# balaji1312/cassnat_asr_public

Measured on AMD Instinct MI355X. Metric: utterances_per_sec, higher is better.
Workload: dtype bf16; 1 GPU; BASELINE configs[1]: CASS-NAT 12L-enc / 1+3+2 dec blocks, d_model 256, 4 heads, d_ff 2048, V 5000, greedy NAST; 32 utterances x 1000 frames x 80 fbank per GPU per step; batch_per_gpu=32, frames=1000, feat_dim=80, global_batch=32, parallelism=utterance-sharded x1, decode_pipelines_per_gpu=2, batches_per_engine_pass=10, utterances_per_engine_pass=320, row_predictions=208, row_predictions_missed=0

## Files before the change

cassnat_asr_public_amd/csrc/attention.hip:

```cpp
#include <cstdlib>

#include <cstdio>
#include <cstdlib>

#include "kernels.h"

struct AttnParams {
    const unsigned char* Q;
    const unsigned char* K;
    const unsigned char* V;
    void* O;
    long long ldq_b, ldk_b, ldv_b;
    int ldo;
    int H, Lq, Lk;
    const unsigned char* keymask;
    int kv_mod;
    int stamps;
    const int* kv_index;
    const int* klen;
    int o_blk;
    int q_blk, kv_blk;
    int q_col, k_col, v_col, q_n, kv_n;
    const int* kcap;
    int kcap_stride;
    const int* iv;
    int iv_stride;
    int causal;
    float scale;
    const float* rel_pos;
    const float* rel_u;
    const float* rel_v;
    int rel_R, ld_pos;
    const int* row_off;
    int kv_packed;
    const unsigned char* Y;
    const unsigned char* W;
    const float* bt;
};

template <typename T> struct AttnCfg;
template <> struct AttnCfg<bf16> {
    static constexpr int KROW = 128;
    static constexpr int VROW = 192;
    static constexpr int CPR = 8;
    __device__ static int swz(int row) { return (row >> 1) & 7; }
};
template <> struct AttnCfg<float> {
    static constexpr int KROW = 256;
    static constexpr int VROW = 256;
    static constexpr int CPR = 16;
    __device__ static int swz(int row) { return row & 15; }
};

template <> struct AttnCfg<split_t> {
    static constexpr int KROW = 256;
    static constexpr int VROW = 192;
    static constexpr int CPR = 16;
    __device__ static int swz(int row) { return row & 15; }
};

__device__ long long attn_stamps[8];
#define AT_STAMP(i) if (p.stamps && blockIdx.x == 0 && blockIdx.y == gridDim.y - 1 && blockIdx.z == gridDim.z - 1 && threadIdx.x == 0) attn_stamps[i] = (long long)__builtin_amdgcn_s_memtime();

template <typename T, int NW, bool RES, bool REL = false, bool PK = false, bool PROJ = false>
__global__ __launch_bounds__(64 * NW, (RES && NW == 8) ? 4 : ((__is_same(T, split_t) && NW == 4 && !REL) ? 2 : 1)) void attention_kernel(AttnParams p) {
    typedef AttnCfg<T> Cfg;
    typedef typename Frag<T>::type frag_t;
    constexpr bool SPLIT = __is_same(T, split_t);
    static_assert(!SPLIT || !RES, "split-bf16 attention: the staged forms only");
    static_assert(!PROJ || (RES && NW == 8 && !REL && !PK && sizeof(T) == 2), "the projecting form: resident, 8 waves, 16-bit operands");
    constexpr int KROW = Cfg::KROW, CPR = Cfg::CPR;
    constexpr int VROW = RES ? 128 : Cfg::VROW;
    constexpr int KT_BYTES = 64 * KROW, VT_BYTES = (SPLIT ? 2 : 1) * 64 * VROW, NRES = RES ? 4 : 1;
    constexpr int NF = SPLIT ? 4 : KROW / 32;
    constexpr int NT = 64 * NW;
    constexpr int ST_IT = 64 * CPR / NT;

    __shared__ __attribute__((aligned(16))) unsigned char Ks_all[NRES * KT_BYTES];
    __shared__ __attribute__((aligned(16))) unsigned char Vs_all[NRES * VT_BYTES];
    __shared__ __attribute__((aligned(16))) unsigned int Ms_all[NRES * 16];
    __shared__ unsigned int Mplain[NRES];

    const int tid = threadIdx.x, lane = tid & 63, wave = tid >> 6;
    const int half = lane >> 5, l31 = lane & 31;
    int b = blockIdx.z, h = blockIdx.y;
    if constexpr (PROJ) {
        const int id = blockIdx.y + 4 * blockIdx.z, grp = id >> 5, r = id & 31;
        if (grp < ((int)gridDim.z >> 3)) {
            b = grp * 8 + (r & 7);
            h = r >> 3;
        }
    }
    AT_STAMP(0)
    const long long q0 = PK ? (long long)p.row_off[b] : (long long)b * p.Lq;
    const int Lq = PK ? p.row_off[b + 1] - p.row_off[b] : p.Lq;
    if constexpr (PK) {
        if ((int)blockIdx.x * (32 * NW) >= Lq) return;
    }
    const int q_row = blockIdx.x * (32 * NW) + wave * 32 + l31;
    const bool wave_active = (blockIdx.x * (32 * NW) + wave * 32) < Lq;
    const int qc = q_row < Lq ? q_row : Lq - 1;

    frag_t qf[NF];
    {
        const unsigned char* qp = p.Q + (q0 + qc) * p.ldq_b + (long long)h * KROW;
        if constexpr (PROJ) {
            (void)qp;
        } else if constexpr (SPLIT) {
#pragma unroll
            for (int s = 0; s < NF; ++s) {
                const unsigned char* c = qp + (s >> 1) * 128 + (2 * (s & 1) + half) * 16;
                qf[s].hi = as_frag<bf16>(ld16(c));
                qf[s].lo = as_frag<bf16>(ld16(c + 64));
            }
        } else if constexpr (PK) {
            const long long qm = q0 + qc;
#pragma unroll
            for (int s = 0; s < NF; ++s) {
                const unsigned char* src = qp + (2 * s + half) * 16;
                src = p.q_blk ? p.Q + cn_blk16_off(qm, p.q_col + h * 64 + (2 * s + half) * 8, p.q_n) : src;
                qf[s] = as_frag<T>(ld16(src));
            }
        } else if (p.q_blk) {
            const long long qm = q0 + qc;
#pragma unroll
            for (int s = 0; s < NF; ++s) qf[s] = as_frag<T>(ld16(p.Q + cn_blk16_off(qm, p.q_col + h * 64 + (2 * s + half) * 8, p.q_n)));
        } else {
#pragma unroll
            for (int s = 0; s < NF; ++s) qf[s] = as_frag<T>(ld16(qp + (2 * s + half) * 16));
        }
    }
    if constexpr (PROJ) {
        typedef unsigned u32x4 __attribute__((ext_vector_type(4)));
        const long long ym = q0 + qc;
        int y_half = half;
        asm volatile("" : "+v"(y_half));
        const int y_lane = ((y_half << 5) + (int)(ym & 31)) * 16;
        const unsigned char* yb = p.Y + (ym >> 5) * 16384 + y_lane;
        const int key = wave * 32 + l31;
        bf16x8 yf[16];
#pragma unroll
        for (int ks = 0; ks < 16; ++ks) yf[ks] = as_frag<bf16>(ld16(yb + ks * 1024));
        uint4 wr[4];
        auto fetch = [&](int tile) {
            const uint4* src = reinterpret_cast<const uint4*>(p.W) + (long long)tile * 1024 + tid;
#pragma unroll
            for (int i = 0; i < 4; ++i) wr[i] = src[NT * i];
        };
        auto put = [&]() {
#pragma unroll
            for (int i = 0; i < 4; ++i) st16(Ks_all + (tid + NT * i) * 16, wr[i]);
        };
        auto project = [&](int tile, int d, u32x4& o_0, u32x4& o_1) {
            f32x16 a;
#pragma unroll
            for (int g = 0; g < 4; ++g) {
                const f32x4 v = *reinterpret_cast<const f32x4*>(p.bt + 32 * tile + 8 * g + 4 * half);
#pragma unroll
                for (int e = 0; e < 4; ++e) a[4 * g + e] = v[e];
            }
#pragma unroll
            for (int ks = 0; ks < 16; ++ks)
                a = CN_MFMA16(as_frag<bf16>(ld16(Ks_all + d * 16384 + ks * 1024 + lane * 16)), yf[ks], a, 0, 0, 0);
#pragma unroll
            for (int gp = 0; gp < 2; ++gp) {
                bf16x4 o0, o1;
#pragma unroll
                for (int e = 0; e < 4; ++e) {
                    o0[e] = (bf16)a[8 * gp + e];
                    o1[e] = (bf16)a[8 * gp + 4 + e];
                }
                const uint2 lo_ = __builtin_bit_cast(uint2, o0), hi_ = __builtin_bit_cast(uint2, o1);
                const auto s0_ = __builtin_amdgcn_permlane32_swap(lo_.x, hi_.x, false, false);
                const auto s1_ = __builtin_amdgcn_permlane32_swap(lo_.y, hi_.y, false, false);
                (gp ? o_1 : o_0) = u32x4{s0_[0], s1_[0], s0_[1], s1_[1]};
            }
        };
        u32x4 pk[4];
        fetch(16 + 2 * h);
        put();
        __syncthreads();
#pragma unroll
        for (int d = 0; d < 2; ++d) {
            project(16 + 2 * h + d, d, pk[0], pk[1]);
#pragma unroll
            for (int c = 0; c < 2; ++c)
                *reinterpret_cast<u32x4*>(Vs_all + key * 128 + (((2 * (2 * d + c) + half) ^ (((key >> 1) & 1) << 2)) << 4)) = pk[c];
        }
        __syncthreads();
        fetch(2 * h);
        put();
        __syncthreads();
#pragma unroll
        for (int d = 0; d < 2; ++d) {
            project(2 * h + d, d, pk[0], pk[1]);
            qf[2 * d] = __builtin_bit_cast(bf16x8, pk[0]);
            qf[2 * d + 1] = __builtin_bit_cast(bf16x8, pk[1]);
        }
        __syncthreads();
        fetch(8 + 2 * h);
        put();
        __syncthreads();
        project(8 + 2 * h, 0, pk[0], pk[1]);
        project(8 + 2 * h + 1, 1, pk[2], pk[3]);
        __syncthreads();
#pragma unroll
        for (int c = 0; c < 4; ++c)
            *reinterpret_cast<u32x4*>(Ks_all + key * KROW + (((2 * c + half) ^ Cfg::swz(key)) << 4)) = pk[c];
        AT_STAMP(1)
    }
    constexpr int REL_N = REL ? 64 : 1;
    __shared__ float rel_tab[REL ? 64 * 64 : 1];
    __shared__ float rel_bias[REL ? NW : 1][32][REL_N];
    if constexpr (REL) {
        constexpr int E = SPLIT ? 8 : Frag<T>::ELEMS;
        const int nr = 2 * p.rel_R + 1;
        for (int i = tid; i < nr * 64; i += NT) rel_tab[i] = p.rel_pos[(long long)(i >> 6) * p.ld_pos + h * 64 + (i & 63)];
        __syncthreads();
        auto dim_of = [&](int s, int j) -> int {
            if constexpr (SPLIT) return 32 * (s >> 1) + 16 * (s & 1) + 8 * half + j;
            else return (2 * s + half) * E + j;
        };
        float qv[NF][E];
#pragma unroll
        for (int s = 0; s < NF; ++s)
#pragma unroll
            for (int j = 0; j < E; ++j) {
                const int dim = dim_of(s, j);
                if constexpr (SPLIT) {
                    const float q = (float)qf[s].hi[j] + (float)qf[s].lo[j];
                    qv[s][j] = q + p.rel_v[h * 64 + dim];
                    const float qu = q + p.rel_u[h * 64 + dim];
                    const bf16 hi = (bf16)qu;
                    qf[s].hi[j] = hi;
                    qf[s].lo[j] = (bf16)(qu - (float)hi);
                } else {
                    const float q = to_f32(qf[s][j]);
                    qv[s][j] = q + p.rel_v[h * 64 + dim];
                    qf[s][j] = from_f32<T>(q + p.rel_u[h * 64 + dim]);
                }
            }
        for (int r = 0; r < nr; ++r) {
            float acc = 0.f;
#pragma unroll
            for (int s = 0; s < NF; ++s)
#pragma unroll
                for (int j = 0; j < E; ++j) acc = fmaf(qv[s][j], rel_tab[r * 64 + dim_of(s, j)], acc);
            acc += __shfl_xor(acc, 32);
            if (half == 0) rel_bias[wave][l31][r] = acc;
        }
        __syncthreads();
    }
    int iv_s1 = 0, iv_e1 = 0, iv_s2 = 0, iv_e2 = 0;
    if (p.iv) {
        const int4 r = *reinterpret_cast<const int4*>(p.iv + ((long long)b * p.iv_stride + qc) * 4);
        iv_s1 = r.x;
        iv_e1 = r.y;
        iv_s2 = r.z;
        iv_e2 = r.w;
    }
    const int klen = p.klen ? p.klen[b] : p.Lk;
    unsigned char* Ks = Ks_all;
    unsigned char* Vs = Vs_all;
    unsigned int* Ms = Ms_all;

    uint4 k_reg[ST_IT], v_reg[ST_IT];
    const int bk = p.kv_index ? p.kv_index[b] : (p.kv_mod > 0 ? b % p.kv_mod : b);
    const bool kpk = PK && p.kv_packed;
    const long long k0 = kpk ? (long long)p.row_off[bk] : (long long)bk * p.Lk;
    const int krows = kpk ? p.row_off[bk + 1] - p.row_off[bk] : p.Lk;
    int kcap = p.kcap ? p.kcap[(long long)bk * p.kcap_stride] : p.Lk;
    if (krows < kcap) kcap = krows;
    const int kvalid = kcap < p.Lk ? kcap : p.Lk;
    const int nkt = kvalid > 0 ? (kvalid + 63) / 64 : 1;
    const unsigned char* kbase = p.K + k0 * p.ldk_b + (long long)h * KROW;
    const unsigned char* vbase = p.V + k0 * p.ldv_b + (long long)h * KROW;
    auto load_tile = [&](int kt) {
#pragma unroll
        for (int i = 0; i < ST_IT; ++i) {
            const int cidx = tid + NT * i;
            const int row = cidx / CPR, ch = cidx % CPR;
            const int key = kt * 64 + row;
            if (key < krows) {
                if (p.kv_blk) {
                    const long long km = k0 + key;
                    k_reg[i] = ld16(p.K + cn_blk16_off(km, p.k_col + h * 64 + ch * 8, p.kv_n));
                    v_reg[i] = ld16(p.V + cn_blk16_off(km, p.v_col + h * 64 + ch * 8, p.kv_n));
                } else {
                    k_reg[i] = ld16(kbase + (long long)key * p.ldk_b + ch * 16);
                    v_reg[i] = ld16(vbase + (long long)key * p.ldv_b + ch * 16);
                }
            } else {
                k_reg[i] = make_uint4(0, 0, 0, 0);
                v_reg[i] = make_uint4(0, 0, 0, 0);
            }
        }
    };
    auto store_tile = [&](int kt) {
#pragma unroll
        for (int i = 0; i < ST_IT; ++i) {
            const int cidx = tid + NT * i;
            const int row = cidx / CPR, ch = cidx % CPR;
            st16(Ks + row * KROW + ((ch ^ Cfg::swz(row)) << 4), k_reg[i]);
            if constexpr (SPLIT)
                st16(Vs + ((ch >> 2) & 1) * 64 * VROW + row * VROW + ((((ch >> 3) << 2) | (ch & 3)) << 4), v_reg[i]);
            else
                st16(Vs + row * VROW + (ch << 4), v_reg[i]);
        }
        if (tid < 64) {
            const int key = kt * 64 + tid;
            unsigned char code = 2;
            if (key < kcap) {
                bool ok = key < klen;
                if (p.keymask) ok = ok && p.keymask[(long long)bk * p.Lk + key] != 0;
                code = ok ? 1 : 0;
            }
            reinterpret_cast<unsigned char*>(Ms)[tid] = code;
            const unsigned long long bad0 = __ballot(code == 0), bad2 = __ballot(code == 2);
            if (tid == 0) Mplain[0] = 1u | (bad2 != 0ull ? 2u : 0u) | (bad0 != 0ull ? 4u : 0u);
        }
    };

    f32x16 o_acc[2];
#pragma unroll
    for (int d = 0; d < 2; ++d)
#pragma unroll
        for (int r = 0; r < 16; ++r) o_acc[d][r] = 0.f;
    float m_run = CN_NEG_FILL, l_run = 0.f;

    if constexpr (RES) {
        const int wave_u = __builtin_amdgcn_readfirstlane(wave);
        const int r8 = lane >> 3, cp = lane & 7;
        for (int piece = wave_u; !PROJ && piece < nkt * 16; piece += NW) {
            const int kt2 = piece >> 4, is_v = (piece >> 3) & 1, j = piece & 7;
            const int row = 8 * j + r8;
            int key = kt2 * 64 + row;
            if (key >= krows) key = krows - 1;
            const int chunk = is_v ? (cp ^ (((row >> 1) & 1) << 2)) : (cp ^ Cfg::swz(row));
            const unsigned char* src;
            if (p.kv_blk)
                src = (is_v ? p.V : p.K) + cn_blk16_off(k0 + key, (is_v ? p.v_col : p.k_col) + h * 64 + chunk * 8, p.kv_n);
            else
                src = is_v ? vbase + (long long)key * p.ldv_b + (chunk << 4) : kbase + (long long)key * p.ldk_b + (chunk << 4);
            unsigned char* dst = (is_v ? Vs_all + kt2 * VT_BYTES : Ks_all + kt2 * KT_BYTES) + j * 1024;
            __builtin_amdgcn_global_load_lds((const __attribute__((address_space(1))) void*)src,
                                             (__attribute__((address_space(3))) void*)dst, 16, 0, 0);
        }
        if constexpr (!PROJ) AT_STAMP(1)
        if (tid < NRES) Mplain[tid] = 1;
        __syncthreads();
        for (int i = tid; i < nkt * 64; i += NT) {
            unsigned char code = 2;
            if (i < kcap) {
                bool ok = i < klen;
                if (p.keymask) ok = ok && p.keymask[(long long)bk * p.Lk + i] != 0;
                code = ok ? 1 : 0;
            }
            reinterpret_cast<unsigned char*>(Ms_all)[i] = code;
            if (code != 1) atomicOr(&Mplain[i >> 6], code == 2 ? 2u : 4u);
        }
        asm volatile("s_waitcnt vmcnt(0)" ::: "memory");
        __syncthreads();
        AT_STAMP(2)
    } else {
        load_tile(0);
    }
    for (int kt = 0; kt < nkt; ++kt) {
        if constexpr (RES) {
            Ks = Ks_all + kt * KT_BYTES;
            Vs = Vs_all + kt * VT_BYTES;
            Ms = Ms_all + kt * 16;
        } else {
            __syncthreads();
            store_tile(kt);
            __syncthreads();
            if (kt + 1 < nkt) load_tile(kt + 1);
        }
        if (!wave_active) continue;

        const unsigned tile_class = Mplain[RES ? kt : 0];
        const bool simple = !REL && !p.iv && !p.causal && (tile_class & 4u) == 0;
#pragma unroll
        for (int sub = 0; sub < 2; ++sub) {
            if (simple && kt * 64 + sub * 32 >= kcap) continue;
            f32x16 sc;
#pragma unroll
            for (int r = 0; r < 16; ++r) sc[r] = 0.f;
            {
                const int row = sub * 32 + l31;
#pragma unroll
                for (int s = 0; s < NF; ++s) {
                    if constexpr (SPLIT) {
                        const int chunk = (s >> 1) * 8 + 2 * (s & 1) + half;
                        split_frag kf;
                        kf.hi = as_frag<bf16>(ld16(Ks + row * KROW + ((chunk ^ Cfg::swz(row)) << 4)));
                        kf.lo = as_frag<bf16>(ld16(Ks + row * KROW + (((chunk + 4) ^ Cfg::swz(row)) << 4)));
                        sc = mfma_frag(kf, qf[s], sc);
                    } else {
                        const int chunk = 2 * s + half;
                        const frag_t kf = as_frag<T>(ld16(Ks + row * KROW + ((chunk ^ Cfg::swz(row)) << 4)));
                        sc = mfma_frag(kf, qf[s], sc);
                    }
                }
            }
            float psum = 0.f, alpha;
            const bool plain = simple && kt * 64 + sub * 32 + 32 <= kcap;
            if (simple) {
                float tmax;
                if (plain) {
                    tmax = sc[0];
#pragma unroll
                    for (int r = 1; r < 16; ++r) tmax = fmaxf(tmax, sc[r]);
                } else {
                    const int k0 = kt * 64 + sub * 32 + 4 * half;
                    tmax = -INFINITY;
#pragma unroll
                    for (int r = 0; r < 16; ++r) {
                        sc[r] = k0 + 8 * (r >> 2) + (r & 3) < kcap ? sc[r] : -INFINITY;
                        tmax = fmaxf(tmax, sc[r]);
                    }
                }
                tmax = xhalf_max(tmax) * p.scale;
                const float m_new = fmaxf(m_run, tmax);
                alpha = __expf(m_run - m_new);
                m_run = m_new;
                const float c2 = p.scale * 1.44269504088896340736f, mb = m_new * 1.44269504088896340736f;
#pragma unroll
                for (int r = 0; r < 16; ++r) {
                    const float pv = __builtin_amdgcn_exp2f(fmaf(sc[r], c2, -mb));
                    sc[r] = pv;
                    psum += pv;
                }
            } else {
                float tmax = -INFINITY;
#pragma unroll
                for (int g = 0; g < 4; ++g) {
                    const unsigned int mw = Ms[sub * 8 + 2 * g + half];
#pragma unroll
                    for (int e = 0; e < 4; ++e) {
                        const int r = 4 * g + e;
                        const int key = kt * 64 + sub * 32 + 8 * g + 4 * half + e;
                        const unsigned int code = (mw >> (8 * e)) & 0xffu;
                        bool ok = code == 1u;
                        if (p.iv) ok = ok && ((key >= iv_s1 && key < iv_e1) || (key >= iv_s2 && key < iv_e2));
                        if (p.causal) ok = ok && key <= q_row;
                        float v = sc[r];
                        if constexpr (REL) {
                            int rd = key - q_row;
                            rd = rd < -p.rel_R ? -p.rel_R : (rd > p.rel_R ? p.rel_R : rd);
                            v += rel_bias[wave][l31][rd + p.rel_R];
                        }
                        v = ok ? v : CN_NEG_FILL;
                        v = code == 2u ? -INFINITY : v;
                        sc[r] = v;
                        tmax = fmaxf(tmax, ok ? v * p.scale : v);
                    }
                }
                tmax = xhalf_max(tmax);
                const float m_new = fmaxf(m_run, tmax);
                alpha = __expf(m_run - m_new);
                m_run = m_new;
                const float c2 = p.scale * 1.44269504088896340736f, mb = m_new * 1.44269504088896340736f;
                const float p_fill = __expf(CN_NEG_FILL - m_new);
#pragma unroll
                for (int r = 0; r < 16; ++r) {
                    const float v = sc[r];
                    float pv = __builtin_amdgcn_exp2f(fmaf(v, c2, -mb));
                    pv = v == CN_NEG_FILL ? p_fill : pv;
                    pv = v == -INFINITY ? 0.f : pv;
                    sc[r] = pv;
                    psum += pv;
                }
            }
            l_run = l_run * alpha + psum;
            if (!__all(alpha == 1.f)) {
#pragma unroll
                for (int d = 0; d < 2; ++d)
#pragma unroll
                    for (int r = 0; r < 16; ++r) o_acc[d][r] *= alpha;
            }

            if constexpr (SPLIT) {
                const int i16 = lane & 15, g1 = (lane >> 4) & 1;
                typedef short s16x8 __attribute__((ext_vector_type(8)));
#pragma unroll
                for (int s = 0; s < 2; ++s) {
                    bf16x8 ph, pl;
#pragma unroll
                    for (int j = 0; j < 8; ++j) {
                        ph[j] = (bf16)sc[8 * s + j];
                        pl[j] = (bf16)(sc[8 * s + j] - (float)ph[j]);
                    }
                    const int key0 = sub * 32 + 16 * s + 4 * half + (i16 >> 2);
#pragma unroll
                    for (int d = 0; d < 2; ++d) {
                        bf16x8 vf[2];
#pragma unroll
                        for (int pl_ = 0; pl_ < 2; ++pl_) {
                            const unsigned char* a1 = Vs + pl_ * 64 * VROW + key0 * VROW + (32 * d + 16 * g1 + 4 * (i16 & 3)) * 2;
                            const s16x4 r1 = __builtin_amdgcn_ds_read_tr16_b64_v4i16((s16x4 __attribute__((address_space(3)))*)(a1));
                            const s16x4 r2 = __builtin_amdgcn_ds_read_tr16_b64_v4i16((s16x4 __attribute__((address_space(3)))*)(a1 + 8 * VROW));
                            s16x8 cat;
                            cat[0] = r1[0]; cat[1] = r1[1]; cat[2] = r1[2]; cat[3] = r1[3];
                            cat[4] = r2[0]; cat[5] = r2[1]; cat[6] = r2[2]; cat[7] = r2[3];
                            vf[pl_] = __builtin_bit_cast(bf16x8, cat);
                        }
                        o_acc[d] = CN_MFMA16(vf[1], ph, o_acc[d], 0, 0, 0);
                        o_acc[d] = CN_MFMA16(vf[0], pl, o_acc[d], 0, 0, 0);
                        o_acc[d] = CN_MFMA16(vf[0], ph, o_acc[d], 0, 0, 0);
                    }
                }
            } else if constexpr (sizeof(T) == 2) {
                const int i16 = lane & 15, g1 = (lane >> 4) & 1;
#pragma unroll
                for (int s = 0; s < 2; ++s) {
                    bf16x8 pb;
#pragma unroll
                    for (int j = 0; j < 8; ++j) pb[j] = (bf16)sc[8 * s + j];
                    const int key0 = sub * 32 + 16 * s + 4 * half + (i16 >> 2);
#pragma unroll
                    for (int d = 0; d < 2; ++d) {
                        const int dd = RES ? (d ^ ((i16 >> 3) & 1)) : d;
                        const unsigned char* a1 = Vs + key0 * VROW + (32 * dd + 16 * g1 + 4 * (i16 & 3)) * 2;
                        const s16x4 r1 = __builtin_amdgcn_ds_read_tr16_b64_v4i16(
                            (s16x4 __attribute__((address_space(3)))*)(a1));
                        const s16x4 r2 = __builtin_amdgcn_ds_read_tr16_b64_v4i16(
                            (s16x4 __attribute__((address_space(3)))*)(a1 + 8 * VROW));
                        typedef short s16x8 __attribute__((ext_vector_type(8)));
                        s16x8 cat;
                        cat[0] = r1[0]; cat[1] = r1[1]; cat[2] = r1[2]; cat[3] = r1[3];
                        cat[4] = r2[0]; cat[5] = r2[1]; cat[6] = r2[2]; cat[7] = r2[3];
                        const bf16x8 vf = __builtin_bit_cast(bf16x8, cat);
                        o_acc[d] = CN_MFMA16(vf, pb, o_acc[d], 0, 0, 0);
                    }
                }
            } else {
#pragma unroll
                for (int r = 0; r < 16; ++r) {
                    const int key_local = sub * 32 + acc_row(r, lane);
                    const float* vrow = reinterpret_cast<const float*>(Vs + key_local * VROW);
#pragma unroll
                    for (int d = 0; d < 2; ++d)
                        o_acc[d] = __builtin_amdgcn_mfma_f32_32x32x2f32(vrow[32 * d + l31], sc[r], o_acc[d], 0, 0, 0);
                }
            }
        }
    }

    AT_STAMP(3)
    if (!wave_active) return;
    const float l_tot = xhalf_sum(l_run);
    const float inv = (REL && m_run == CN_NEG_FILL) ? 0.f : 1.f / l_tot;
    if constexpr (sizeof(T) == 2) {
        typedef unsigned u32x4 __attribute__((ext_vector_type(4)));
        T* orow = reinterpret_cast<T*>(p.O) + (q0 + qc) * p.ldo + h * 64 + 8 * half;
#pragma unroll
        for (int d = 0; d < 2; ++d) {
#pragma unroll
            for (int gp = 0; gp < 2; ++gp) {
                bf16x4 o0, o1;
#pragma unroll
                for (int e = 0; e < 4; ++e) {
                    o0[e] = (bf16)(o_acc[d][8 * gp + e] * inv);
                    o1[e] = (bf16)(o_acc[d][8 * gp + 4 + e] * inv);
                }
                const uint2 lo_ = __builtin_bit_cast(uint2, o0), hi_ = __builtin_bit_cast(uint2, o1);
                const auto s0_ = __builtin_amdgcn_permlane32_swap(lo_.x, hi_.x, false, false);
                const auto s1_ = __builtin_amdgcn_permlane32_swap(lo_.y, hi_.y, false, false);
                if (q_row < Lq) {
                    if (p.o_blk) {
                        const long long om = q0 + q_row;
                        unsigned char* ob = reinterpret_cast<unsigned char*>(p.O) +
                                            ((om >> 5) * (p.ldo >> 4) + (4 * h + 2 * d + gp)) * 1024 + ((half << 5) + (int)(om & 31)) * 16;
                        *reinterpret_cast<u32x4*>(ob) = u32x4{s0_[0], s1_[0], s0_[1], s1_[1]};
                    } else {
                        *reinterpret_cast<u32x4*>(orow + 32 * d + 16 * gp) = u32x4{s0_[0], s1_[0], s0_[1], s1_[1]};
                    }
                }
            }
        }
        return;
    }
    if (q_row < Lq) {
        T* orow = reinterpret_cast<T*>(p.O) + (q0 + q_row) * p.ldo + h * 64;
#pragma unroll
        for (int d = 0; d < 2; ++d) {
#pragma unroll
            for (int g = 0; g < 4; ++g) {
                const int dk0 = 32 * d + 8 * g + 4 * half;
                if constexpr (SPLIT) {
                    float o[4];
#pragma unroll
                    for (int e = 0; e < 4; ++e) o[e] = o_acc[d][4 * g + e] * inv;
                    bf16x4 hi, lo;
                    cn_split4(o, hi, lo);
                    unsigned char* ob = reinterpret_cast<unsigned char*>(orow) + cn_split_off((size_t)dk0);
                    *reinterpret_cast<bf16x4*>(ob) = hi;
                    *reinterpret_cast<bf16x4*>(ob + 64) = lo;
                } else if constexpr (sizeof(T) == 2) {
                    bf16x4 o;
#pragma unroll
                    for (int e = 0; e < 4; ++e) o[e] = (bf16)(o_acc[d][4 * g + e] * inv);
                    *reinterpret_cast<bf16x4*>(orow + dk0) = o;
                } else {
                    f32x4 o;
#pragma unroll
                    for (int e = 0; e < 4; ++e) o[e] = o_acc[d][4 * g + e] * inv;
                    *reinterpret_cast<f32x4*>(orow + dk0) = o;
                }
            }
        }
    }
    AT_STAMP(4)
}

int attention_print_stamps() {
    long long h[8];
    CN_HIP_CHECK(hipMemcpyFromSymbol(h, HIP_SYMBOL(attn_stamps), sizeof(h)));
    static const char* names[] = {"", "Q fragments + K/V requests", "K/V landed + mask codes", "key-tile loop", "normalise + store"};
    for (int i = 1; i < 5; ++i) fprintf(stderr, "[attention stamps] %-28s %8lld ticks\n", names[i], h[i] - h[i - 1]);
    fprintf(stderr, "[attention stamps] total %lld ticks (s_memtime)\n", h[4] - h[0]);
    return 0;
}

template <typename T> static int run_attention(const AttnArgs& a, hipStream_t s) {
    constexpr bool PKT = sizeof(T) == 2 && !__is_same(T, split_t);
    AttnParams p;
    p.Q = (const unsigned char*)a.Q;
    p.K = (const unsigned char*)a.K;
    p.V = (const unsigned char*)a.V;
    p.O = a.O;
    p.ldq_b = (long long)a.ldq * sizeof(T);
    p.ldk_b = (long long)a.ldk * sizeof(T);
    p.ldv_b = (long long)a.ldv * sizeof(T);
    p.ldo = a.ldo;
    p.H = a.H;
    p.Lq = a.Lq;
    p.Lk = a.Lk;
    p.keymask = a.keymask;
    p.kv_mod = a.kv_mod;
    static const int stamps = cn_exp_env("CASSNAT_ATTN_STAMPS") ? 1 : 0;
    p.stamps = stamps;
    p.kv_index = a.kv_index;
    p.klen = a.klen;
    p.kcap = a.kcap;
    p.kcap_stride = a.kcap_stride;
    p.o_blk = a.o_blocked;
    p.q_blk = a.q_blocked;
    p.kv_blk = a.kv_blocked;
    p.q_col = a.q_col;
    p.k_col = a.k_col;
    p.v_col = a.v_col;
    p.q_n = a.q_n;
    p.kv_n = a.kv_n;
    if ((a.q_blocked || a.kv_blocked || a.o_blocked) && (sizeof(T) != 2 || __is_same(T, split_t) || a.rel_pos || (a.q_blocked && a.q_n % 32) ||
                                          (a.kv_blocked && a.kv_n % 32) || (a.o_blocked && a.ldo % 32))) {
        cn_set_error("attention: blocked operands exist for the bf16 kernels without relative positions; column counts % 32 == 0");
        return -1;
    }
    p.row_off = a.row_off;
    p.kv_packed = a.kv_packed;
    p.Y = (const unsigned char*)a.proj_y;
    p.W = (const unsigned char*)a.proj_w;
    p.bt = a.proj_b;
    if ((a.row_off && (a.rel_pos || sizeof(T) != 2 || __is_same(T, split_t))) ||
        (a.kv_packed && (!a.row_off || a.kv_mod > 0 || a.kv_index || a.keymask || a.Lq != a.Lk))) {
        cn_set_error("attention: packed rows exist for the 16-bit kernels without relative positions; packed keys are the entry's own "
                     "rows (self attention without a key mask, kv_mod or kv_index)");
        return -1;
    }
    p.iv = a.intervals;
    p.iv_stride = a.iv_stride;
    p.causal = a.causal;
    p.scale = a.scale;
    p.rel_pos = a.rel_pos;
    p.rel_u = a.rel_u;
    p.rel_v = a.rel_v;
    p.rel_R = a.rel_R;
    p.ld_pos = a.ld_pos;
    {
        if (a.rel_pos) {
            if (a.rel_R < 0 || a.rel_R > 31 || !a.rel_u || !a.rel_v || a.Lq != a.Lk) {
                cn_set_error("attention: relative positions need self attention and max_relative_len <= 31");
                return -1;
            }
            hipLaunchKernelGGL((attention_kernel<T, 2, false, true>), dim3(cn_ceil_div(a.Lq, 64), a.H, a.B), dim3(128), 0, s, p);
            CN_HIP_CHECK(hipGetLastError());
            return 0;
        }
    }
    if (a.proj_y) {
        if constexpr (sizeof(T) == 2) {
            if (!a.proj_w || !a.proj_b || a.H != 4 || a.Lq != a.Lk || a.Lk > 256 || a.row_off || a.rel_pos || a.kv_mod > 0 || a.kv_index) {
                cn_set_error("attention: the projecting form is self attention of at most 256 rows per entry, 4 heads (d_model 256), "
                             "without packed rows, relative positions, kv_mod or kv_index");
                return -1;
            }
            hipLaunchKernelGGL((attention_kernel<T, 8, true, false, false, true>), dim3(1, a.H, a.B), dim3(512), 0, s, p);
            CN_HIP_CHECK(hipGetLastError());
            return 0;
        } else {
            cn_set_error("attention: the projecting form exists for the 16-bit kernels");
            return -1;
        }
    }
    const long long big_grid = (long long)cn_ceil_div(a.Lq, 128) * a.H * a.B;
    if constexpr (sizeof(T) == 2) {
        static const int no_res = cn_exp_env("CASSNAT_ATTN_NO_RES") ? 1 : 0;
        if (a.Lk <= 256 && !no_res) {
            static const int nw = cn_exp_env("CASSNAT_ATTN_NW") ? atoi(cn_exp_env("CASSNAT_ATTN_NW")) : 0;
            const int use = nw ? nw : (a.Lq > 128 ? 8 : (a.Lq > 64 ? 4 : 2));
            if (a.row_off) {
                if (use >= 8)
                    hipLaunchKernelGGL((attention_kernel<T, 8, true, false, PKT>), dim3(cn_ceil_div(a.Lq, 256), a.H, a.B), dim3(512), 0, s, p);
                else if (use >= 4)
                    hipLaunchKernelGGL((attention_kernel<T, 4, true, false, PKT>), dim3(cn_ceil_div(a.Lq, 128), a.H, a.B), dim3(256), 0, s, p);
                else
                    hipLaunchKernelGGL((attention_kernel<T, 2, true, false, PKT>), dim3(cn_ceil_div(a.Lq, 64), a.H, a.B), dim3(128), 0, s, p);
            } else if (use >= 8)
                hipLaunchKernelGGL((attention_kernel<T, 8, true>), dim3(cn_ceil_div(a.Lq, 256), a.H, a.B), dim3(512), 0, s, p);
            else if (use >= 4)
                hipLaunchKernelGGL((attention_kernel<T, 4, true>), dim3(cn_ceil_div(a.Lq, 128), a.H, a.B), dim3(256), 0, s, p);
            else
                hipLaunchKernelGGL((attention_kernel<T, 2, true>), dim3(cn_ceil_div(a.Lq, 64), a.H, a.B), dim3(128), 0, s, p);
            CN_HIP_CHECK(hipGetLastError());
            return 0;
        }
    }
    if (a.row_off) {
        if (big_grid >= 1024)
            hipLaunchKernelGGL((attention_kernel<T, 4, false, false, PKT>), dim3(cn_ceil_div(a.Lq, 128), a.H, a.B), dim3(256), 0, s, p);
        else
            hipLaunchKernelGGL((attention_kernel<T, 2, false, false, PKT>), dim3(cn_ceil_div(a.Lq, 64), a.H, a.B), dim3(128), 0, s, p);
    } else if (big_grid >= 1024)
        hipLaunchKernelGGL((attention_kernel<T, 4, false>), dim3(cn_ceil_div(a.Lq, 128), a.H, a.B), dim3(256), 0, s, p);
    else
        hipLaunchKernelGGL((attention_kernel<T, 2, false>), dim3(cn_ceil_div(a.Lq, 64), a.H, a.B), dim3(128), 0, s, p);
    CN_HIP_CHECK(hipGetLastError());
    return 0;
}

int launch_attention(int prec, const AttnArgs& a, hipStream_t s) {
    if (a.B <= 0 || a.Lq <= 0 || a.Lk <= 0 || a.H <= 0) return 0;
    const size_t es = cn_elem_size(prec);
    if ((a.ldq * es) % 16 || (a.ldk * es) % 16 || (a.ldv * es) % 16 || (a.ldo * es) % 16) {
        cn_set_error("attention: row strides must keep rows 16-byte aligned");
        return -1;
    }
    if (prec == CN_PREC_X3) {
        if (a.ldq % 32 || a.ldk % 32 || a.ldv % 32 || a.ldo % 32) {
            cn_set_error("attention: split-bf16 rows need strides that are multiples of 32 elements");
            return -1;
        }
    }
    const long long w = 64LL * a.H;
    const bool qkv_used = a.proj_y == nullptr;
    if ((qkv_used && ((!a.q_blocked && a.ldq < w) || (!a.kv_blocked && (a.ldk < w || a.ldv < w)))) || a.ldo < w) {
        cn_set_error("attention: row strides ldq / ldk / ldv / ldo must be >= 64 * H");
        return -1;
    }
    if (a.rel_pos && a.ld_pos < w) {
        cn_set_error("attention: the relative-position table needs ld_pos >= 64 * H");
        return -1;
    }
    auto bad_window = [w](int col, int n) { return col < 0 || col % 8 || col + w > n; };
    if ((a.q_blocked && bad_window(a.q_col, a.q_n)) ||
        (a.kv_blocked && (bad_window(a.k_col, a.kv_n) || bad_window(a.v_col, a.kv_n)))) {
        cn_set_error("attention: a blocked operand's columns col .. col + 64 * H - 1 must lie inside its q_n / kv_n columns "
                     "(col >= 0, col % 8 == 0)");
        return -1;
    }
// ... 4 lines not shown
```

cassnat_asr_public_amd/csrc/ops.hip:

```cpp
#include <algorithm>
#include <cmath>
#include <cstring>
#include <string>
#include <thread>
#include <vector>

#include "../../include/cassnat_hip.h"
#include "../../include/cassnat_hip_attention_proj.h"
#include "ctc_bias_search.h"
#include "ctc_ngram_search.h"
#include "ctc_times_search.h"
#include "edit_align_search.h"
#include "flac_decode.h"
#include "kernels.h"

namespace {

class Scratch {
  public:
    Scratch(const char* who, hipStream_t s) : who_(who), s_(s) {}
    Scratch(const Scratch&) = delete;
    Scratch& operator=(const Scratch&) = delete;
    ~Scratch() {
        (void)hipStreamSynchronize(s_);
// ... 671 lines not shown
        return -1;
    }
    CN_TRY(conv_module_dims("cn_op_dwconv", precision, B, L, d, "L * d (or B * L)"));
    if ((long long)d * k > 0x7fffffffLL || (long long)L + k > 0x7fffffffLL) {
        cn_set_error("cn_op_dwconv: d * k and L + k exceed the kernels' int arithmetic (<= 2^31 - 1)");
        return -1;
    }
    return launch_dwconv(precision, x, w, bias, y, B, L, d, k, form, (hipStream_t)stream);
}

extern "C" int cn_op_groupnorm_swish(int32_t precision, const float* x, double* stats, const float* gw, const float* gb, void* out,
                                     int32_t B, int32_t L, int32_t d, float eps, void* stream) {
    if ((precision = cn_own_precision(precision, "cn_op_groupnorm_swish")) < 0) return -1;
    if (!x || !stats || !gw || !gb || !out) {
        cn_set_error("cn_op_groupnorm_swish: null pointer (x, stats, gw, gb, out)");
        return -1;
    }
    if (B < 1 || L < 1 || d < 1) {
        cn_set_error("cn_op_groupnorm_swish: B, L and d must be >= 1");
        return -1;
    }
    CN_TRY(conv_module_dims("cn_op_groupnorm_swish", precision, B, L, d, "L * d (or B * L)"));
    return launch_groupnorm_swish(precision, x, stats, gw, gb, out, B, L, d, eps, (hipStream_t)stream);
}

extern "C" int cn_op_attention(int32_t precision, const void* Q, int32_t ldq, const void* K, int32_t ldk, const void* V,
                               int32_t ldv, void* O, int32_t ldo, int32_t B, int32_t H, int32_t Lq, int32_t Lk,
                               const uint8_t* keymask, const int32_t* klen, const int32_t* intervals, int32_t iv_stride,
                               int32_t causal, float scale, void* stream) {
    if ((precision = cn_own_precision(precision, "cn_op_attention")) < 0) return -1;
    AttnArgs a;
    a.Q = Q;
    a.K = K;
    a.V = V;
    a.O = O;
    a.ldq = ldq;
    a.ldk = ldk;
    a.ldv = ldv;
    a.ldo = ldo;
    a.B = B;
    a.H = H;
    a.Lq = Lq;
    a.Lk = Lk;
    a.keymask = keymask;
    a.klen = klen;
    a.intervals = intervals;
    a.iv_stride = iv_stride;
    a.causal = causal;
    a.scale = scale;
    int rc = launch_attention(precision, a, (hipStream_t)stream);
    if (rc == 0 && cn_exp_env("CASSNAT_ATTN_STAMPS")) {
        (void)hipStreamSynchronize((hipStream_t)stream);
        (void)attention_print_stamps();
    }
    return rc;
}

static int op_attention_desc(const char* who, int32_t precision, const cn_attn_desc* d, const int32_t* row_off, int32_t kv_packed,
                             void* stream) {
    if ((precision = cn_own_precision(precision, who)) < 0) return -1;
    if (!d) {
        cn_set_error(std::string(who) + ": null descriptor");
        return -1;
    }
    AttnArgs a;
    a.row_off = row_off;
    a.kv_packed = kv_packed;
    a.Q = d->Q;
    a.K = d->K;
    a.V = d->V;
    a.O = d->O;
    a.ldq = d->ldq;
    a.ldk = d->ldk;
    a.ldv = d->ldv;
    a.ldo = d->ldo;
    a.B = d->B;
    a.H = d->H;
    a.Lq = d->Lq;
    a.Lk = d->Lk;
    a.keymask = d->keymask;
    a.kv_mod = d->kv_mod;
    a.kv_index = d->kv_index;
    a.klen = d->klen;
    a.kcap = d->kcap;
    a.kcap_stride = d->kcap_stride;
    a.q_blocked = d->q_blocked;
    a.kv_blocked = d->kv_blocked;
    a.q_col = d->q_col;
    a.k_col = d->k_col;
    a.v_col = d->v_col;
    a.q_n = d->q_n;
    a.kv_n = d->kv_n;
    a.o_blocked = d->o_blocked;
    a.intervals = d->intervals;
    a.iv_stride = d->iv_stride;
    a.causal = d->causal;
    a.scale = d->scale;
    a.rel_pos = d->rel_pos;
    a.rel_u = d->rel_u;
    a.rel_v = d->rel_v;
    a.rel_R = d->rel_R;
    a.ld_pos = d->ld_pos;
    return launch_attention(precision, a, (hipStream_t)stream);
}

extern "C" int cn_op_attention_desc(int32_t precision, const cn_attn_desc* d, void* stream) {
    return op_attention_desc("cn_op_attention_desc", precision, d, nullptr, 0, stream);
}

extern "C" int cn_op_attention_proj(int32_t precision, const cn_attn_desc* d, const void* y_dev, const float* wt_host,
                                    const float* bt_host, void* stream) {
    if ((precision = cn_own_precision(precision, "cn_op_attention_proj")) < 0) return -1;
    if (!d || !y_dev || !wt_host || !bt_host) {
        cn_set_error("cn_op_attention_proj: null argument");
        return -1;
    }
    if (precision != CN_PREC_BF16) {
        cn_set_error("cn_op_attention_proj: the projecting form exists for the 16-bit kernels");
        return -1;
    }
    ChainWeights w;
    w.wt = wt_host;
    w.bt = bt_host;
    w.tail_n = 768;
    std::vector<uint16_t> hs(chain_stream_units(0, 0, 768) * (CHAIN_UNIT_BYTES / 2));
    std::vector<float> ht(CHAIN_TAB_FLOATS);
    pack_chain(w, hs.data(), ht.data());
    Scratch sc("cn_op_attention_proj", (hipStream_t)stream);
    const void* ds = sc.upload(hs.data(), hs.size() * 2);
    const float* dt = (const float*)sc.upload(ht.data(), ht.size() * 4);
    if (!sc.ok()) return -2;
    AttnArgs a;
    a.O = d->O;
    a.ldo = d->ldo;
    a.B = d->B;
    a.H = d->H;
    a.Lq = d->Lq;
    a.Lk = d->Lk;
    a.keymask = d->keymask;
    a.kv_mod = d->kv_mod;
    a.kv_index = d->kv_index;
    a.klen = d->klen;
    a.kcap = d->kcap;
    a.kcap_stride = d->kcap_stride;
    a.o_blocked = d->o_blocked;
    a.intervals = d->intervals;
    a.iv_stride = d->iv_stride;
    a.causal = d->causal;
    a.scale = d->scale;
    a.rel_pos = d->rel_pos;
    a.proj_y = y_dev;
    a.proj_w = ds;
    a.proj_b = dt + CHAIN_TAB_BT;
    return sc.finish(launch_attention(precision, a, (hipStream_t)stream));
}

extern "C" int cn_op_attention_packed(int32_t precision, const cn_attn_desc* d, const int32_t* row_off_dev, int32_t kv_packed,
                                      void* stream) {
    if (!row_off_dev) {
        cn_set_error("cn_op_attention_packed: null row_off");
        return -1;
    }
    return op_attention_desc("cn_op_attention_packed", precision, d, row_off_dev, kv_packed, stream);
}

extern "C" int cn_op_row_plan(const int32_t* ylen_dev, int32_t B, int32_t U, int32_t hyp_stride, int32_t sub, const int32_t* utt_meta_dev,
                              const int32_t* ymax_dev, int32_t* row_off_dev, void* stream) {
    static_assert(sizeof(UttMeta) == 4 * sizeof(int32_t), "cn_op_row_plan: utt_meta is [B][4] int32");
    if (!ylen_dev || !row_off_dev || B < 1 || U < 0 || sub < 0) {
        cn_set_error("cn_op_row_plan: null argument or B < 1");
        return -1;
    }
    return launch_row_plan(ylen_dev, B, U, hyp_stride, sub, reinterpret_cast<const UttMeta*>(utt_meta_dev), ymax_dev, row_off_dev,
                           (hipStream_t)stream);
}

extern "C" int32_t cn_attn_desc_size(void) { return (int32_t)sizeof(cn_attn_desc); }

extern "C" int cn_op_logsoftmax_argmax(float* logits, int32_t M, int32_t V, int32_t* arg, float* maxlp,
                                       int32_t write_logp, void* stream) {
    return launch_logsoftmax_argmax(logits, M, V, V, arg, maxlp, write_logp, (hipStream_t)stream);
}

extern "C" int cn_op_ctc_align(const int32_t* best, const uint8_t* keymask, const float* size_ratio, int32_t B,
                               int32_t Tp, int32_t blank, int32_t left, int32_t right, int32_t* shift,
                               int32_t* src_size, int32_t* ylen, int32_t* ymax, int32_t* intervals, void* stream) {
    AlignArgs a;
    a.best = best;
    a.keymask = keymask;
    a.size_ratio = size_ratio;
    a.B = B;
    a.Tp = Tp;
    a.blank = blank;
    a.left = left;
    a.right = right;
    a.shift = shift;
    a.src_size = src_size;
    a.ylen = ylen;
    a.ymax = ymax;
    a.intervals = intervals;
    return launch_ctc_align(a, (hipStream_t)stream);
}

extern "C" int cn_op_ctc_prefix_beam(const float* logp, const float* size_ratio, int32_t B, int32_t Tp, int32_t V, int32_t beam,
                                     int32_t pruning, double length_penalty, int32_t blank, int32_t* hyp, int32_t hyp_cap,
                                     int32_t* hyp_len, double* score, double* p_blk, double* p_nblk, int32_t* nbeam, void* stream) {
    hipStream_t s = (hipStream_t)stream;
    const size_t M = (size_t)B * Tp;
    const int P = pruning > 0 ? pruning : 1;
    Scratch sc("cn_op_ctc_prefix_beam", s);
    int* top_idx = (int*)sc.alloc(M * P * 4);
    float* top_val = (float*)sc.alloc(M * P * 4);
    unsigned char* hpar = (unsigned char*)sc.alloc(M * (size_t)std::max(beam, 1));
    int* htok = (int*)sc.alloc(M * (size_t)std::max(beam, 1) * 4);
    if (!sc.ok()) return -2;
    int rc = pruning > 0 ? launch_topk(logp, (int)M, V, V, pruning, top_idx, top_val, s) : 0;
    if (rc == 0) {
        CtcBeamArgs a = ctc_beam_args(logp, top_idx, size_ratio, B, Tp, V, beam, pruning, blank, length_penalty,
                                      ctc_beam_out(hyp, hyp_cap, hyp_len, score, nullptr, p_blk, p_nblk, nbeam));
        a.hist_parent = hpar;
        a.hist_tok = htok;
        rc = launch_ctc_prefix_beam(a, s);
    }
    return sc.finish(rc);
}

extern "C" int cn_op_ctc_viterbi(const float* logp, const uint8_t* keymask, const float* size_ratio, const int32_t* labels,
                                 const int32_t* label_len, int32_t B, int32_t Tp, int32_t V, int32_t ld, int32_t ymax, int32_t blank,
                                 int32_t* out_path, void* stream) {
    hipStream_t s = (hipStream_t)stream;
    Scratch sc("cn_op_ctc_viterbi", s);
    unsigned char* bp = (unsigned char*)sc.alloc((size_t)B * Tp * (2 * (size_t)ymax + 1));
    if (!sc.ok()) return -2;
    ViterbiArgs v;
    v.logp = logp;
    v.keymask = keymask;
    v.size_ratio = size_ratio;
    v.labels = labels;
    v.label_len = label_len;
    v.B = B;
    v.Tp = Tp;
    v.V = V;
    v.ld = ld;
    v.ymax = ymax;
    v.blank = blank;
    v.bp = bp;
    v.out_path = out_path;
    return sc.finish(launch_ctc_viterbi(v, s));
}

extern "C" int cn_op_ctc_token_times(const float* logp_dev, const int32_t* frames_dev, const int32_t* labels_dev, int32_t ld,
                                     const int32_t* label_len_dev, int32_t B, int32_t Tp, int32_t V, int32_t blank, int64_t bp_lds_limit,
                                     int32_t* start_dev, int32_t* end_dev, float* conf_dev, double* score_dev, int32_t* status_dev,
                                     void* stream) {
    CtcTimesArgs a;
    a.logp = logp_dev, a.frames = frames_dev, a.labels = labels_dev, a.label_len = label_len_dev;
    a.B = B, a.Tp = Tp, a.V = V, a.ld = ld, a.blank = blank;
    a.start = start_dev, a.end = end_dev, a.conf = conf_dev, a.score = score_dev, a.status = status_dev;
    const std::string bad = ct_check(a);
    if (!bad.empty()) {
        cn_set_error("cn_op_ctc_token_times: " + bad);
        return -1;
    }
    hipStream_t s = (hipStream_t)stream;
    Scratch sc("cn_op_ctc_token_times", s);
    if (const size_t need = ct_scratch_bytes(B, Tp, ld, bp_lds_limit)) a.bp = (unsigned long long*)sc.alloc(need);
    if (!sc.ok()) return -2;
    return sc.finish(launch_ctc_token_times(a, bp_lds_limit, s));
}

extern "C" int cn_op_edit_align(const int32_t* ref_dev, int64_t ref_total, const int64_t* ref_begin_dev, const int32_t* ref_len_dev,
                                const int32_t* hyp_dev, int64_t hyp_total, const int64_t* hyp_begin_dev, const int32_t* hyp_len_dev, int32_t N,
                                int32_t max_ref, int32_t max_hyp, int32_t c_sub, int32_t c_ins, int32_t c_del, int64_t bp_lds_limit,
                                int32_t* cost_dev, int32_t* counts_dev, int32_t* path_len_dev, uint8_t* ops_dev, int64_t ops_total,
                                const int64_t* ops_begin_dev, void* stream) {
    EditArgs a;
    a.ref = ref_dev, a.ref_begin = ref_begin_dev, a.ref_len = ref_len_dev, a.hyp = hyp_dev, a.hyp_begin = hyp_begin_dev, a.hyp_len = hyp_len_dev;
    a.ops_begin = ops_begin_dev, a.ref_total = ref_total, a.hyp_total = hyp_total, a.ops_total = ops_total;
    a.N = N, a.max_ref = max_ref, a.max_hyp = max_hyp, a.c_sub = c_sub, a.c_ins = c_ins, a.c_del = c_del;
    a.cost = cost_dev, a.counts = counts_dev, a.path_len = path_len_dev, a.ops = ops_dev;
    const std::string bad = ea_check(a);
    if (!bad.empty()) {
        cn_set_error("cn_op_edit_align: " + bad);
        return -1;
    }
    hipStream_t s = (hipStream_t)stream;
    Scratch sc("cn_op_edit_align", s);
    if (const size_t need = ea_scratch_bytes(N, max_ref, max_hyp, bp_lds_limit)) a.bp = (unsigned long long*)sc.alloc(need);
    if (!sc.ok()) return -2;
    return sc.finish(launch_edit_align(a, bp_lds_limit, s));
}

extern "C" int cn_op_greedy_pack(const int32_t* tok, const float* val, const int32_t* ylen, int32_t B, int32_t U,
                                 int32_t sos, int32_t hyp_stride, int32_t* hyp, int32_t* hyp_len, double* score,
                                 void* stream) {
    return launch_greedy_pack(tok, val, ylen, B, U, sos, hyp_stride, hyp, hyp_len, score, (hipStream_t)stream);
}

extern "C" int cn_op_topk(const float* logp, int32_t M, int32_t V, int32_t k, int32_t* idx, float* val, void* stream) {
    return launch_topk(logp, M, V, V, k, idx, val, (hipStream_t)stream);
}

extern "C" int cn_op_gemm_fp8(const void* a_bf16_dev, int32_t lda, const float* w_host, const float* bias_dev, float* c_dev,
                              int32_t M, int32_t N, int32_t K, float a_scale, int32_t relu, float* w_scale_out, void* stream) {
    if (M < 1 || N < 1 || K < 128 || K % 128 != 0) {
        cn_set_error("cn_op_gemm_fp8: K must be a positive multiple of 128");
        return -1;
// ... 1041 lines not shown
```

Baseline: 53480 utt/s.

## Stage all projection weight tiles into LDS up front and precompute key mask

The projecting attention prologue used to fetch three weight regions serially through registers, storing each into LDS between barriers. It now issues all five 16-KiB weight units at once with direct global-to-LDS loads into Ks/Vs and an enlarged Ms slot, reorders the Q/K/V projections to drop barriers, and loads the key mask, klen and kcap early, computing per-tile mask classes with wave ballots instead of atomics. This hides global latency behind the projection MFMAs. The cost is more LDS per workgroup, which may lower occupancy. Optional stamp printing is also added, off by default.

```diff
diff --git a/cassnat_asr_public_amd/csrc/attention.hip b/cassnat_asr_public_amd/csrc/attention.hip
--- a/cassnat_asr_public_amd/csrc/attention.hip
+++ b/cassnat_asr_public_amd/csrc/attention.hip
@@ -59,7 +59,7 @@
     __device__ static int swz(int row) { return row & 15; }
 };
 
-__device__ long long attn_stamps[8];
+__device__ long long attn_stamps[16];
 #define AT_STAMP(i) if (p.stamps && blockIdx.x == 0 && blockIdx.y == gridDim.y - 1 && blockIdx.z == gridDim.z - 1 && threadIdx.x == 0) attn_stamps[i] = (long long)__builtin_amdgcn_s_memtime();
 
 template <typename T, int NW, bool RES, bool REL = false, bool PK = false, bool PROJ = false>
@@ -78,8 +78,12 @@
 
     __shared__ __attribute__((aligned(16))) unsigned char Ks_all[NRES * KT_BYTES];
     __shared__ __attribute__((aligned(16))) unsigned char Vs_all[NRES * VT_BYTES];
-    __shared__ __attribute__((aligned(16))) unsigned int Ms_all[NRES * 16];
+    constexpr int PROJ_SLOT = 16384;
+    __shared__ __attribute__((aligned(16))) unsigned int Ms_all[PROJ ? PROJ_SLOT / 4 : NRES * 16];
     __shared__ unsigned int Mplain[NRES];
+    static_assert(!PROJ || (sizeof(Ks_all) + sizeof(Vs_all) + sizeof(Ms_all) == 81920 && sizeof(Ks_all) == 2 * PROJ_SLOT && sizeof(Vs_all) == 2 * PROJ_SLOT),
+                  "the projecting form: five 16-KiB slots, half of a CU's LDS");
+    constexpr int PROJ_CLASS = NRES * 16;
 
     const int tid = threadIdx.x, lane = tid & 63, wave = tid >> 6;
     const int half = lane >> 5, l31 = lane & 31;
@@ -130,6 +134,8 @@
             for (int s = 0; s < NF; ++s) qf[s] = as_frag<T>(ld16(qp + (2 * s + half) * 16));
         }
     }
+    unsigned long long pj_km = 0;
+    int pj_klen = 0, pj_kcap = 0;
     if constexpr (PROJ) {
         typedef unsigned u32x4 __attribute__((ext_vector_type(4)));
         const long long ym = q0 + qc;
@@ -138,20 +144,34 @@
         const int y_lane = ((y_half << 5) + (int)(ym & 31)) * 16;
         const unsigned char* yb = p.Y + (ym >> 5) * 16384 + y_lane;
         const int key = wave * 32 + l31;
+        unsigned char* const slotA = Ks_all;
+        unsigned char* const slotB = Vs_all;
+        unsigned char* const slotC = reinterpret_cast<unsigned char*>(Ms_all);
+        const unsigned char* wh = p.W + (long long)h * (2 * PROJ_SLOT);
+        {
+            const int wave_u = __builtin_amdgcn_readfirstlane(wave);
+#pragma unroll
+            for (int i = 0; i < 10; ++i) {
+                const int region = i >> 2;
+                const int piece = wave_u + 8 * i - 32 * region;
+                const unsigned char* src = wh + (region == 0 ? 16 : (region == 1 ? 8 : 0)) * PROJ_SLOT + piece * 1024 + lane * 16;
+                unsigned char* dst = (region == 0 ? slotA : (region == 1 ? slotB : slotC)) + piece * 1024;
+                __builtin_amdgcn_global_load_lds((const __attribute__((address_space(1))) void*)src,
+                                                 (__attribute__((address_space(3))) void*)dst, 16, 0, 0);
+            }
+        }
+        uint4 wq[2];
+#pragma unroll
+        for (int i = 0; i < 2; ++i) wq[i] = reinterpret_cast<const uint4*>(wh + PROJ_SLOT)[tid + NT * i];
         bf16x8 yf[16];
 #pragma unroll
         for (int ks = 0; ks < 16; ++ks) yf[ks] = as_frag<bf16>(ld16(yb + ks * 1024));
-        uint4 wr[4];
-        auto fetch = [&](int tile) {
-            const uint4* src = reinterpret_cast<const uint4*>(p.W) + (long long)tile * 1024 + tid;
-#pragma unroll
-            for (int i = 0; i < 4; ++i) wr[i] = src[NT * i];
-        };
-        auto put = [&]() {
-#pragma unroll
-            for (int i = 0; i < 4; ++i) st16(Ks_all + (tid + NT * i) * 16, wr[i]);
-        };
-        auto project = [&](int tile, int d, u32x4& o_0, u32x4& o_1) {
+        const unsigned char* km_src = p.keymask ? p.keymask + (long long)b * p.Lk + (tid < p.Lk ? tid : 0) : p.W;
+        const int* klen_src = p.klen ? p.klen + b : reinterpret_cast<const int*>(p.W);
+        const int* kcap_src = p.kcap ? p.kcap + (long long)b * p.kcap_stride : reinterpret_cast<const int*>(p.W);
+        const unsigned char km_raw = *km_src;
+        const int klen_raw = *klen_src, kcap_raw = *kcap_src;
+        auto project = [&](int tile, const unsigned char* unit, u32x4& o_0, u32x4& o_1) {
             f32x16 a;
 #pragma unroll
             for (int g = 0; g < 4; ++g) {
@@ -161,7 +181,7 @@
             }
 #pragma unroll
             for (int ks = 0; ks < 16; ++ks)
-                a = CN_MFMA16(as_frag<bf16>(ld16(Ks_all + d * 16384 + ks * 1024 + lane * 16)), yf[ks], a, 0, 0, 0);
+                a = CN_MFMA16(as_frag<bf16>(ld16(unit + ks * 1024 + lane * 16)), yf[ks], a, 0, 0, 0);
 #pragma unroll
             for (int gp = 0; gp < 2; ++gp) {
                 bf16x4 o0, o1;
@@ -176,34 +196,36 @@
                 (gp ? o_1 : o_0) = u32x4{s0_[0], s1_[0], s0_[1], s1_[1]};
             }
         };
-        u32x4 pk[4];
-        fetch(16 + 2 * h);
-        put();
+        u32x4 pk[4], pv[2];
+        asm volatile("s_waitcnt vmcnt(0)" ::: "memory");
         __syncthreads();
+        pj_km = __ballot(!p.keymask || tid >= p.Lk || km_raw != 0);
+        pj_klen = p.klen ? __builtin_amdgcn_readfirstlane(klen_raw) : p.Lk;
+        pj_kcap = p.kcap ? __builtin_amdgcn_readfirstlane(kcap_raw) : p.Lk;
+        AT_STAMP(8)
+        project(2 * h, slotC, pv[0], pv[1]);
+        qf[0] = __builtin_bit_cast(bf16x8, pv[0]);
+        qf[1] = __builtin_bit_cast(bf16x8, pv[1]);
+        __syncthreads();
+        AT_STAMP(9)
+#pragma unroll
+        for (int i = 0; i < 2; ++i) st16(slotC + (tid + NT * i) * 16, wq[i]);
+        project(8 + 2 * h, slotB, pk[0], pk[1]);
+        project(8 + 2 * h + 1, slotB + PROJ_SLOT, pk[2], pk[3]);
+        __syncthreads();
+        AT_STAMP(10)
 #pragma unroll
         for (int d = 0; d < 2; ++d) {
-            project(16 + 2 * h + d, d, pk[0], pk[1]);
+            project(16 + 2 * h + d, slotA + d * PROJ_SLOT, pv[0], pv[1]);
 #pragma unroll
             for (int c = 0; c < 2; ++c)
-                *reinterpret_cast<u32x4*>(Vs_all + key * 128 + (((2 * (2 * d + c) + half) ^ (((key >> 1) & 1) << 2)) << 4)) = pk[c];
-        }
+                *reinterpret_cast<u32x4*>(Vs_all + key * 128 + (((2 * (2 * d + c) + half) ^ (((key >> 1) & 1) << 2)) << 4)) = pv[c];
+        }
+        project(2 * h + 1, slotC, pv[0], pv[1]);
+        qf[2] = __builtin_bit_cast(bf16x8, pv[0]);
+        qf[3] = __builtin_bit_cast(bf16x8, pv[1]);
         __syncthreads();
-        fetch(2 * h);
-        put();
-        __syncthreads();
-#pragma unroll
-        for (int d = 0; d < 2; ++d) {
-            project(2 * h + d, d, pk[0], pk[1]);
-            qf[2 * d] = __builtin_bit_cast(bf16x8, pk[0]);
-            qf[2 * d + 1] = __builtin_bit_cast(bf16x8, pk[1]);
-        }
-        __syncthreads();
-        fetch(8 + 2 * h);
-        put();
-        __syncthreads();
-        project(8 + 2 * h, 0, pk[0], pk[1]);
-        project(8 + 2 * h + 1, 1, pk[2], pk[3]);
-        __syncthreads();
+        AT_STAMP(11)
 #pragma unroll
         for (int c = 0; c < 4; ++c)
             *reinterpret_cast<u32x4*>(Ks_all + key * KROW + (((2 * c + half) ^ Cfg::swz(key)) << 4)) = pk[c];
@@ -259,7 +281,7 @@
         iv_s2 = r.z;
         iv_e2 = r.w;
     }
-    const int klen = p.klen ? p.klen[b] : p.Lk;
+    const int klen = PROJ ? pj_klen : (p.klen ? p.klen[b] : p.Lk);
     unsigned char* Ks = Ks_all;
     unsigned char* Vs = Vs_all;
     unsigned int* Ms = Ms_all;
@@ -269,7 +291,7 @@
     const bool kpk = PK && p.kv_packed;
     const long long k0 = kpk ? (long long)p.row_off[bk] : (long long)bk * p.Lk;
     const int krows = kpk ? p.row_off[bk + 1] - p.row_off[bk] : p.Lk;
-    int kcap = p.kcap ? p.kcap[(long long)bk * p.kcap_stride] : p.Lk;
+    int kcap = PROJ ? pj_kcap : (p.kcap ? p.kcap[(long long)bk * p.kcap_stride] : p.Lk);
     if (krows < kcap) kcap = krows;
     const int kvalid = kcap < p.Lk ? kcap : p.Lk;
     const int nkt = kvalid > 0 ? (kvalid + 63) / 64 : 1;
@@ -346,22 +368,34 @@
             __builtin_amdgcn_global_load_lds((const __attribute__((address_space(1))) void*)src,
                                              (__attribute__((address_space(3))) void*)dst, 16, 0, 0);
         }
-        if constexpr (!PROJ) AT_STAMP(1)
-        if (tid < NRES) Mplain[tid] = 1;
-        __syncthreads();
-        for (int i = tid; i < nkt * 64; i += NT) {
-            unsigned char code = 2;
-            if (i < kcap) {
-                bool ok = i < klen;
-                if (p.keymask) ok = ok && p.keymask[(long long)bk * p.Lk + i] != 0;
-                code = ok ? 1 : 0;
-            }
-            reinterpret_cast<unsigned char*>(Ms_all)[i] = code;
-            if (code != 1) atomicOr(&Mplain[i >> 6], code == 2 ? 2u : 4u);
-        }
-        asm volatile("s_waitcnt vmcnt(0)" ::: "memory");
-        __syncthreads();
-        AT_STAMP(2)
+        if constexpr (PROJ) {
+            if (tid < 64 * NRES) {
+                unsigned char code = 2;
+                if (tid < kcap) code = (tid < klen && ((pj_km >> lane) & 1ull) != 0) ? 1 : 0;
+                reinterpret_cast<unsigned char*>(Ms_all)[tid] = code;
+                const unsigned long long bad0 = __ballot(code == 0), bad2 = __ballot(code == 2);
+                if (lane == 0) Ms_all[PROJ_CLASS + wave] = 1u | (bad2 != 0ull ? 2u : 0u) | (bad0 != 0ull ? 4u : 0u);
+            }
+            __syncthreads();
+            AT_STAMP(2)
+        } else {
+            AT_STAMP(1)
+            if (tid < NRES) Mplain[tid] = 1;
+            __syncthreads();
+            for (int i = tid; i < nkt * 64; i += NT) {
+                unsigned char code = 2;
+                if (i < kcap) {
+                    bool ok = i < klen;
+                    if (p.keymask) ok = ok && p.keymask[(long long)bk * p.Lk + i] != 0;
+                    code = ok ? 1 : 0;
+                }
+                reinterpret_cast<unsigned char*>(Ms_all)[i] = code;
+                if (code != 1) atomicOr(&Mplain[i >> 6], code == 2 ? 2u : 4u);
+            }
+            asm volatile("s_waitcnt vmcnt(0)" ::: "memory");
+            __syncthreads();
+            AT_STAMP(2)
+        }
     } else {
         load_tile(0);
     }
@@ -378,7 +412,9 @@
         }
         if (!wave_active) continue;
 
-        const unsigned tile_class = Mplain[RES ? kt : 0];
+        unsigned tile_class;
+        if constexpr (PROJ) tile_class = Ms_all[PROJ_CLASS + kt];
+        else tile_class = Mplain[RES ? kt : 0];
         const bool simple = !REL && !p.iv && !p.causal && (tile_class & 4u) == 0;
 #pragma unroll
         for (int sub = 0; sub < 2; ++sub) {
@@ -615,8 +651,16 @@
 }
 
 int attention_print_stamps() {
-    long long h[8];
+    long long h[16];
     CN_HIP_CHECK(hipMemcpyFromSymbol(h, HIP_SYMBOL(attn_stamps), sizeof(h)));
+    if (h[8] > h[0] && h[11] < h[1]) {
+        static const char* pn[] = {"rows, five units, key mask landed", "Q tile 0 projected", "Q unit 1 staged, K projected", "V, Q tile 1 projected"};
+        for (int i = 8; i < 12; ++i) fprintf(stderr, "[attention stamps] prologue: %-34s %8lld ticks\n", pn[i - 8], h[i] - (i == 8 ? h[0] : h[i - 1]));
+        fprintf(stderr, "[attention stamps] prologue: %-34s %8lld ticks\n", "K image written", h[1] - h[11]);
+        int per_cu = 0;
+        CN_HIP_CHECK(hipOccupancyMaxActiveBlocksPerMultiprocessor(&per_cu, attention_kernel<bf16, 8, true, false, false, true>, 512, 0));
+        fprintf(stderr, "[attention stamps] prologue: the runtime places %d workgroups of the projecting form on a CU\n", per_cu);
+    }
     static const char* names[] = {"", "Q fragments + K/V requests", "K/V landed + mask codes", "key-tile loop", "normalise + store"};
     for (int i = 1; i < 5; ++i) fprintf(stderr, "[attention stamps] %-28s %8lld ticks\n", names[i], h[i] - h[i - 1]);
     fprintf(stderr, "[attention stamps] total %lld ticks (s_memtime)\n", h[4] - h[0]);
diff --git a/cassnat_asr_public_amd/csrc/ops.hip b/cassnat_asr_public_amd/csrc/ops.hip
--- a/cassnat_asr_public_amd/csrc/ops.hip
+++ b/cassnat_asr_public_amd/csrc/ops.hip
@@ -847,7 +847,12 @@
     a.proj_y = y_dev;
     a.proj_w = ds;
     a.proj_b = dt + CHAIN_TAB_BT;
-    return sc.finish(launch_attention(precision, a, (hipStream_t)stream));
+    int rc = launch_attention(precision, a, (hipStream_t)stream);
+    if (rc == 0 && cn_exp_env("CASSNAT_ATTN_STAMPS")) {
+        (void)hipStreamSynchronize((hipStream_t)stream);
+        (void)attention_print_stamps();
+    }
+    return sc.finish(rc);
 }
 
 extern "C" int cn_op_attention_packed(int32_t precision, const cn_attn_desc* d, const int32_t* row_off_dev, int32_t kv_packed,
```

Result: no change. 53800 utt/s, median of 6 (+0.6%).
